# element36-io/hyperfridge-r0

Measured on AMD Instinct MI355X. Metric: segments/sec (po2=20) proving camt53 guest, 1/2/4/8 MI355X, higher is better.
Workload: dtype u32

## Files before the change

### hyperfridge-r0_amd/csrc/circuit.hpp

```cpp
#pragma once
#include <mutex>

#include "../../include/r0hip_circuit.h"
#include "internal.hpp"

namespace r0h {

struct Tap { uint32_t group, offset, back; };
struct Reg { uint32_t group, offset, first_tap, size, combo; };
struct Step { uint32_t op, a, b, c; };
struct CodeCol { uint32_t kind, param; };
struct DataCol { uint32_t kind, a, b, c, e; };
struct AccCol { uint32_t first, a, b; };
struct Term { uint32_t pow, v; std::vector<uint32_t> conds; };
struct LfTerm { uint32_t coef, global, col; };
struct Lf { std::vector<LfTerm> terms; };
struct LogupPart { uint32_t ch_kind, ch_idx; Lf lf; };
struct LogupFraction { uint32_t table; Lf num; std::vector<LogupPart> parts; };
struct LogupAcc { uint32_t final_global; std::vector<LogupFraction> fr; };
struct LogupTable { uint32_t data_col, kind; };
struct Logup {
  std::vector<LogupTable> tables;
  std::vector<LogupAcc> accs;
  uint32_t n_chain = 0;
// ... 42 lines not shown
  std::vector<uint32_t> global_cols;
  std::vector<r0h::Step> steps;
  uint32_t ret = 0;
  std::vector<uint32_t> fp_step, mix_step;
  std::vector<r0h::CodeCol> code_cols;
  std::vector<r0h::DataCol> data_cols;
  std::vector<r0h::AccCol> acc_cols;
  r0h::Logup logup;
  uint32_t period = 0;
  std::vector<uint32_t> periodic;
  bool has_sponge = false;
  uint32_t sponge_code = 0, sponge_data = 0, sponge_global = 0;
  uint32_t n_late = 0;
  bool has_column_program = false;
  std::vector<uint32_t> blob;
  uint8_t info[16] = {'R', '0', 'H', 'I', 'P', '_', 'S', 'Y', 'N', 'T', 'H', ':', 'v', '1', '_', '_'};
  r0h::Plan plan;
  hipModule_t module = nullptr;
  std::vector<hipFunction_t> kernels;
  mutable std::mutex check_mu;
  mutable hipModule_t check_module = nullptr;
  mutable std::vector<hipFunction_t> check_kernels;
};

namespace r0h {
const char* parse_blob(r0h_circuit* c, const uint32_t* blob, size_t n_words);
void make_plan(r0h_circuit* c);
std::string emit_source(const r0h_circuit* c);
std::string emit_check_source(const r0h_circuit* c);
const char* sponge_plant(r0h_ctx* ctx, const r0h_circuit* c, uint32_t po2, const uint32_t* words, size_t n_words, r0h_buf* data);
const char* require_witness(const char* caller, r0h_ctx* ctx, const r0h_circuit* c, uint32_t po2, const r0h_buf* accum, const r0h_buf* code, const r0h_buf* data,
                            const uint32_t* global, const uint32_t* mix);
const char* logup_accum(r0h_ctx* ctx, const r0h_circuit* c, uint32_t po2, const r0h_buf* code, const r0h_buf* data, const uint32_t* global, const uint32_t* mix, r0h_buf* accum);
}
```

### hyperfridge-r0_amd/csrc/fp.hpp

```cpp
#pragma once
#include <stdint.h>
#if defined(__HIPCC__)
#include <hip/hip_runtime.h>
#define R0H_HD __host__ __device__ __forceinline__
#else
#define R0H_HD inline
#endif

namespace r0h {

constexpr uint32_t P = 2013265921u;
constexpr uint32_t NPINV = 0x77ffffffu;
constexpr uint32_t R2 = 1172168163u;
constexpr uint32_t ONE = 268435454u;
constexpr uint32_t ROU_GEN = 137u;
constexpr uint32_t BETA_CANON = 11u;

R0H_HD uint32_t reduce1(uint32_t x) {
#if defined(__HIP_DEVICE_COMPILE__)
  uint32_t r;
  asm("v_subrev_co_u32 %0, vcc, 0x78000001, %1\n\tv_cndmask_b32 %0, %0, %1, vcc" : "=&v"(r) : "v"(x) : "vcc");
  return r;
#else
  uint32_t y = x - P;
  return y < x ? y : x;
#endif
}
R0H_HD uint32_t add(uint32_t a, uint32_t b) { return reduce1(a + b); }
R0H_HD uint32_t sub(uint32_t a, uint32_t b) {
#if defined(__HIP_DEVICE_COMPILE__)
  uint32_t d, e;
  asm("v_sub_co_u32 %0, vcc, %2, %3\n\tv_add_u32 %1, 0x78000001, %0\n\tv_cndmask_b32 %0, %0, %1, vcc"
      : "=&v"(d), "=&v"(e) : "v"(a), "v"(b) : "vcc");
  return d;
#else
  uint32_t d = a - b, e = d + P;
  return d < e ? d : e;
#endif
}
// ... 66 lines not shown
  uint32_t c4 = reduce64((u64)a.e[1] * b.e[3] + (u64)a.e[2] * b.e[2] + (u64)a.e[3] * b.e[1]);
  uint32_t c5 = reduce64((u64)a.e[2] * b.e[3] + (u64)a.e[3] * b.e[2]);
  uint32_t c6 = reduce64((u64)a.e[3] * b.e[3]);
  Fp4 r;
  r.e[0] = reduce64((u64)a.e[0] * b.e[0] + (u64)BETA_M * c4);
  r.e[1] = reduce64((u64)a.e[0] * b.e[1] + (u64)a.e[1] * b.e[0] + (u64)BETA_M * c5);
  r.e[2] = reduce64((u64)a.e[0] * b.e[2] + (u64)a.e[1] * b.e[1] + (u64)a.e[2] * b.e[0] + (u64)BETA_M * c6);
  r.e[3] = reduce64((u64)a.e[0] * b.e[3] + (u64)a.e[1] * b.e[2] + (u64)a.e[2] * b.e[1] + (u64)a.e[3] * b.e[0]);
  return r;
}
R0H_HD Fp4 fp4_pow(Fp4 a, uint64_t n) {
  Fp4 r = fp4_one();
  while (n) {
    if (n & 1) r = r * a;
    a = a * a;
    n >>= 1;
  }
  return r;
}
R0H_HD Fp4 fp4_inv(const Fp4& a) {
  uint32_t A0 = a.e[0], A1 = a.e[2], B0 = a.e[1], B1 = a.e[3];
  uint32_t A2_0 = add(mul(A0, A0), mul(BETA_M, mul(A1, A1))), A2_1 = mul(add(A0, A0), A1);
  uint32_t B2_0 = add(mul(B0, B0), mul(BETA_M, mul(B1, B1))), B2_1 = mul(add(B0, B0), B1);
  uint32_t D0 = sub(A2_0, mul(BETA_M, B2_1)), D1 = sub(A2_1, B2_0);
  uint32_t n = inv(sub(mul(D0, D0), mul(BETA_M, mul(D1, D1))));
  uint32_t I0 = mul(D0, n), I1 = neg(mul(D1, n));
  Fp4 r;
  r.e[0] = add(mul(A0, I0), mul(BETA_M, mul(A1, I1)));
  r.e[2] = add(mul(A0, I1), mul(A1, I0));
  r.e[1] = neg(add(mul(B0, I0), mul(BETA_M, mul(B1, I1))));
  r.e[3] = neg(add(mul(B0, I1), mul(B1, I0)));
  return r;
}

R0H_HD uint32_t bitrev(uint32_t x, uint32_t bits) {
#if defined(__HIP_DEVICE_COMPILE__)
  return bits ? __brev(x) >> (32 - bits) : 0u;
#else
  uint32_t r = 0;
  for (uint32_t i = 0; i < bits; i++) r |= ((x >> i) & 1u) << (bits - 1 - i);
  return r;
#endif
}
inline uint32_t rou_fwd(uint32_t po2) { return fpow(enc(ROU_GEN), 1ull << (27 - po2)); }
inline uint32_t rou_rev(uint32_t po2) { return inv(rou_fwd(po2)); }

}
```

### hyperfridge-r0_amd/csrc/internal.hpp

```cpp
#pragma once
#include <hip/hip_runtime.h>
#include <stdint.h>
#include <stdio.h>
#include <stdlib.h>
#include <string.h>

#include <map>
#include <memory>
#include <string>
#include <vector>

#include "../../include/r0hip.h"
#include "fp.hpp"

namespace r0h {

const char* make_error(const char* fmt, ...);

#define R0H_TRY_HIP(expr)                                                                              \
  do {                                                                                                 \
    hipError_t e__ = (expr);                                                                           \
    if (e__ != hipSuccess) return r0h::make_error("%s:%d: %s: %s", __FILE__, __LINE__, #expr, hipGetErrorString(e__)); \
  } while (0)
#define R0H_TRY(expr)                \
// ... 19 lines not shown
constexpr uint32_t TW_TOP = 22;
constexpr uint32_t TWB_BITS = 13;
constexpr uint32_t TWB_SIZE = 1u << TWB_BITS;
constexpr uint32_t MAX_DOMAIN_PO2 = 26;
constexpr size_t POOL_LIMIT = (size_t)192 << 30;

struct P2Consts {
  uint32_t rc_full[2 * P2_HALF_FULL][P2_CELLS];
  uint32_t rc_partial[P2_PARTIAL];
  uint32_t diag[P2_CELLS];
  uint32_t diag_canon[P2_CELLS];
  uint32_t diag_shoup[P2_CELLS];
  uint32_t part_sigma[P2_PART_SIGMA_WORDS];
  uint32_t part_final[(P2_CELLS - 1) * (P2_PARTIAL + 1)];
};

struct KTimer {
  std::vector<hipEvent_t> ev;
  size_t used = 0;
  double alg_bytes = 0;
};

struct Profile {
  std::vector<const char*> names;
  std::vector<float> ms;
  std::vector<hipEvent_t> events;
};

}

struct r0h_ctx {
  int device = 0;
  int refs = 1;

  hipStream_t stream = nullptr;
  uint32_t* tw_lo[2] = {nullptr, nullptr};
  uint32_t* tw_hi[2] = {nullptr, nullptr};
  uint32_t* tw12[2] = {nullptr, nullptr};
  uint32_t* twb_lo[2] = {nullptr, nullptr};
  uint32_t* twb_hi[2] = {nullptr, nullptr};
  uint32_t* pow3_lo = nullptr;
  uint32_t* pow3_hi = nullptr;
  uint32_t* pow3_top = nullptr;
  r0h::P2Consts* p2 = nullptr;
  r0h::P2Consts p2_host;
  int hashfn = 0;
  void* scratch = nullptr;
  size_t scratch_bytes = 0;
  void* pinned = nullptr;
  size_t pinned_bytes = 0, pinned_off = 0;
  std::multimap<size_t, void*> pool;
  size_t pool_bytes = 0;
  r0h::Profile prof;
  r0h_session_stats session = {0, 0, 0, 0, 0, 0, 0};
  const r0h_circuit* image_circuit = nullptr;
  uint64_t session_resident_limit = 0;
  void* session_rows = nullptr;
  std::vector<r0h_ctx*> helpers;
  bool check_witness = false;
  bool ktime_on = false;
  std::map<std::string, r0h::KTimer> ktimers;
};

struct r0h_buf {
  r0h_ctx* ctx = nullptr;
  void* ptr = nullptr;
// ... 94 lines not shown
```

### hyperfridge-r0_amd/csrc/logup.hip

```cpp
#include <algorithm>
#include <map>

#include "../../include/r0hip_circuit.h"
#include "circuit.hpp"

namespace r0h {

namespace {
struct Tape {
  std::vector<uint32_t> words;
  std::vector<const uint32_t*> cols;
  std::vector<Fp4> ch;
  std::vector<uint32_t> acc_begin;
};

const char* build_tape(const r0h_circuit* c, uint32_t po2, const r0h_buf* code, const r0h_buf* data, const uint32_t* global, const uint32_t* mix, Tape* t, bool lookups_only = false) {
  std::map<uint32_t, uint32_t> col_index;
  std::map<uint64_t, uint32_t> ch_index;
  t->ch.push_back(fp4_one());
  auto form = [&](const Lf& lf) -> const char* {
    t->words.push_back((uint32_t)lf.terms.size());
    for (const LfTerm& term : lf.terms) {
      uint32_t coef = enc(term.coef);
      if (term.global) {
        R0H_REQUIRE(global, "log-derivative accumulation: a form reads a public input and none were given");
        coef = mul(coef, global[term.global - 1]);
      }
      uint32_t col = 0;
      if (term.col) {
        const uint32_t ref = term.col - 1;
        auto it = col_index.find(ref);
        if (it == col_index.end()) {
          const r0h_buf* src = (ref >> 28) == R0H_GROUP_CODE ? code : data;
          R0H_REQUIRE(src, "log-derivative accumulation: a form reads the %s group and none was given", (ref >> 28) == R0H_GROUP_CODE ? "CODE" : "DATA");
          it = col_index.emplace(ref, (uint32_t)t->cols.size()).first;
          t->cols.push_back(u32(src) + ((size_t)(ref & 0xfffffu) << po2));
        }
        col = it->second + 1;
      }
      t->words.push_back(coef);
      t->words.push_back(col);
    }
    return nullptr;
  };
  for (const LogupAcc& a : c->logup.accs) {
    t->acc_begin.push_back((uint32_t)t->words.size());
    for (const LogupFraction& f : a.fr) {
      if (lookups_only && !f.table) continue;
      t->words.push_back(f.table);
      R0H_TRY(form(f.num));
      t->words.push_back((uint32_t)f.parts.size());
      for (const LogupPart& q : f.parts) {
        uint32_t idx = 0;
        if (q.ch_kind) {
          const uint64_t key = (uint64_t)q.ch_kind << 32 | q.ch_idx;
          auto it = ch_index.find(key);
          if (it == ch_index.end()) {
            const uint32_t* src = q.ch_kind == 1 ? mix + 4 * (size_t)q.ch_idx : global + q.ch_idx;
            R0H_REQUIRE(q.ch_kind == 1 ? mix != nullptr : global != nullptr, "log-derivative accumulation: a challenge is read from %s and none were given", q.ch_kind == 1 ? "the mix" : "the public inputs");
            it = ch_index.emplace(key, (uint32_t)t->ch.size()).first;
            t->ch.push_back(Fp4{{src[0], src[1], src[2], src[3]}});
          }
          idx = it->second;
        }
        t->words.push_back(idx);
        R0H_TRY(form(q.lf));
      }
    }
  }
  t->acc_begin.push_back((uint32_t)t->words.size());
  return nullptr;
}

struct DeviceTape {
  DevBuf buf;
  const uint32_t* words = nullptr;
  const uint32_t* const* cols = nullptr;
  const Fp4* ch = nullptr;
};
const char* upload_tape(r0h_ctx* ctx, const Tape& t, DeviceTape* d) {
  const size_t w_bytes = (t.words.size() * 4 + 15) & ~(size_t)15, c_bytes = (t.cols.size() * sizeof(void*) + 15) & ~(size_t)15, h_bytes = t.ch.size() * 16;
  R0H_TRY(d->buf.alloc(ctx, w_bytes + c_bytes + h_bytes));
  char* base = (char*)d->buf->ptr;
  R0H_TRY(stage_h2d(ctx, base, t.words.data(), t.words.size() * 4));
  R0H_TRY(stage_h2d(ctx, base + w_bytes, t.cols.data(), t.cols.size() * sizeof(void*)));
  R0H_TRY(stage_h2d(ctx, base + w_bytes + c_bytes, t.ch.data(), h_bytes));
  d->words = (const uint32_t*)base;
  d->cols = (const uint32_t* const*)(base + w_bytes);
  d->ch = (const Fp4*)(base + w_bytes + c_bytes);
  return nullptr;
}

__device__ __forceinline__ uint32_t eval_form(const uint32_t* __restrict__ tape, uint32_t& at, const uint32_t* const* __restrict__ cols, uint32_t r) {
  const uint32_t n = tape[at++];
  uint32_t acc = 0;
  for (uint32_t k = 0; k < n; k++) {
    const uint32_t coef = tape[at], col = tape[at + 1];
    at += 2;
    acc = add(acc, col ? mul(coef, cols[col - 1][r]) : coef);
  }
  return acc;
}

constexpr uint32_t HOT = 4096;

__global__ __launch_bounds__(256) void logup_count_kernel(uint32_t* __restrict__ hist , uint32_t* __restrict__ err, const uint32_t* __restrict__ tape,
                                                          uint32_t tape_end, const uint32_t* const* __restrict__ cols, uint32_t n, uint32_t n_tables) {
  __shared__ uint32_t hot[2][HOT];
  for (uint32_t i = threadIdx.x; i < 2 * HOT; i += 256) (&hot[0][0])[i] = 0;
  __syncthreads();
  const uint32_t r = blockIdx.x * 256u + threadIdx.x;
  uint32_t gated[2] = {0, 0};
  if (r < n) {
    uint32_t at = 0;
    while (at < tape_end) {
      const uint32_t table = tape[at++];
      const uint32_t num = eval_form(tape, at, cols, r);
      const uint32_t n_parts = tape[at++];
      uint32_t value = 0;
      for (uint32_t q = 0; q < n_parts; q++) {
        at++;
        const uint32_t v = eval_form(tape, at, cols, r);
        if (q == 1) value = v;
      }
      if (!table || table > n_tables) continue;
      if (num != ONE) {
        if (num) atomicOr(err, 1u);
        else gated[table - 1]++;
        continue;
      }
      uint32_t v = dec(neg(value));
      if (table == R0H_TABLE_AND) {
        v -= R0H_TAG_AND;
        if (v >> 24 || ((v & 255u) & ((v >> 8) & 255u)) != v >> 16) { atomicOr(err, 2u); continue; }
        v &= 0xffffu;
      } else if (v >> 16) {
        atomicOr(err, 2u);
        continue;
      }
      if (!v) continue;
      if (v < HOT) atomicAdd(&hot[table - 1][v], 1u);
      else atomicAdd(&hist[(size_t)(table - 1) * 65536 + v], 1u);
    }
  }
  if (gated[0]) atomicAdd(&hot[0][0], gated[0]);
  if (gated[1]) atomicAdd(&hot[1][0], gated[1]);
  __syncthreads();
  for (uint32_t i = threadIdx.x; i < 2 * HOT; i += 256) {
    const uint32_t cnt = (&hot[0][0])[i];
    if (cnt) atomicAdd(&hist[(size_t)(i / HOT) * 65536 + (i % HOT)], cnt);
  }
}
__global__ void logup_mult_kernel(uint32_t* __restrict__ column, const uint32_t* __restrict__ hist, uint32_t total, uint32_t n) {
  __shared__ uint32_t part[256];
  const uint32_t r = blockIdx.x * 256u + threadIdx.x;
  if (blockIdx.x == 0) {
    uint32_t s = 0;
    for (uint32_t i = threadIdx.x; i < 65536u; i += 256) s += hist[i];
    part[threadIdx.x] = s;
    __syncthreads();
    for (uint32_t k = 128; k; k >>= 1) {
      if (threadIdx.x < k) part[threadIdx.x] += part[threadIdx.x + k];
      __syncthreads();
    }
  }
  if (r >= n) return;
  uint32_t v = r < 65536u ? hist[r] : 0u;
  if (r == 0) v = total - part[0];
  column[r] = enc(v);
}

__global__ __launch_bounds__(256) void logup_term_kernel(uint32_t* __restrict__ accum, uint32_t* __restrict__ row_total, uint32_t* __restrict__ own_terms,
                                                         const uint32_t* __restrict__ tape, const uint32_t* const* __restrict__ cols, const Fp4* __restrict__ ch,
                                                         uint32_t a0, uint32_t a1, uint32_t n_chain, uint32_t po2) {
  const uint32_t r = blockIdx.x * 256u + threadIdx.x, n = 1u << po2;
  if (r >= n) return;
  uint32_t at = 0;
  Fp4 run = fp4_zero();
  for (uint32_t j = a0; j < a1; j++) {
    Fp4 d[4];
    uint32_t num[4];
    for (uint32_t f = 0; f < 4; f++) {
      at++;
      num[f] = eval_form(tape, at, cols, r);
      const uint32_t n_parts = tape[at++];
      Fp4 den = fp4_zero();
      for (uint32_t q = 0; q < n_parts; q++) {
        const uint32_t ci = tape[at++];
        const uint32_t v = eval_form(tape, at, cols, r);
        if (ci == 0) den.e[0] = add(den.e[0], v);
        else den = den + scale(ch[ci], v);
      }
      d[f] = den;
    }
    const Fp4 d01 = d[0] * d[1], d23 = d[2] * d[3];
    const Fp4 top = (scale(d[1], num[0]) + scale(d[0], num[1])) * d23 + (scale(d[3], num[2]) + scale(d[2], num[3])) * d01;
    const Fp4 term = top * fp4_inv(d01 * d23);
    if (j < n_chain) {
      run = run + term;
      for (uint32_t i = 0; i < 4; i++) accum[((size_t)(4 * j + i) << po2) + r] = run.e[i];
    } else {
      *(uint4*)(own_terms + 4 * ((size_t)(j - n_chain) * n + r)) = make_uint4(term.e[0], term.e[1], term.e[2], term.e[3]);
    }
  }
  if (a0 < n_chain) *(uint4*)(row_total + 4 * (size_t)r) = make_uint4(run.e[0], run.e[1], run.e[2], run.e[3]);
}
__global__ void logup_chain_kernel(uint32_t* __restrict__ accum, const uint32_t* __restrict__ scanned, uint32_t n_cols, uint32_t po2) {
  const uint32_t r = blockIdx.x * 256u + threadIdx.x, col = blockIdx.y;
  if (r == 0 || r >= (1u << po2) || col >= n_cols) return;
  uint32_t* cell = accum + ((size_t)col << po2) + r;
  *cell = add(*cell, scanned[4 * (size_t)(r - 1) + (col & 3u)]);
}
}

static const char* own_accumulators(r0h_ctx* ctx, const r0h_circuit* c, uint32_t po2, const Tape& t, const DeviceTape& d, r0h_buf* accum, uint32_t* totals_out) {
  const uint32_t n = 1u << po2, n_chain = c->logup.n_chain, n_acc = (uint32_t)c->logup.accs.size(), n_own = n_acc - n_chain;
  if (!n_own) return nullptr;
  DevBuf terms;
  R0H_TRY(terms.alloc(ctx, (size_t)n_own * n * 16));
  hipLaunchKernelGGL(logup_term_kernel, dim3((n + 255) / 256), dim3(256), 0, ctx->stream, accum ? u32(accum) : nullptr, (uint32_t*)nullptr, u32(terms.get()),
                     d.words + t.acc_begin[n_chain], d.cols, d.ch, n_chain, n_acc, n_chain, po2);
  R0H_TRY(launch_ok("logup_term_kernel"));
  for (uint32_t k = 0; k < n_own; k++) {
    r0h_buf view = buf_view(terms.get(), (size_t)k * n * 16, (size_t)n * 16);
    R0H_TRY(r0h_prefix_sums(ctx, &view, n));
    if (accum) R0H_TRY(unpack_ext_columns(ctx, u32(accum) + ((size_t)(4 * (n_chain + k)) << po2), (const uint32_t*)view.ptr, po2));
    if (totals_out) R0H_TRY(r0h_buf_d2h(ctx, &view, (size_t)(n - 1) * 16, totals_out + 4 * k, 16));
  }
  return nullptr;
}

const char* logup_accum(r0h_ctx* ctx, const r0h_circuit* c, uint32_t po2, const r0h_buf* code, const r0h_buf* data, const uint32_t* global, const uint32_t* mix, r0h_buf* accum) {
  R0H_GUARD_BEGIN
  R0H_REQUIRE(ctx && c && data && accum, "r0h_accum: NULL argument");
  R0H_REQUIRE(po2 >= 4 && po2 <= R0H_MAX_PO2, "r0h_accum: po2 %u outside [4, %u]", po2, R0H_MAX_PO2);
  const uint32_t n = 1u << po2, n_chain = c->logup.n_chain;
  R0H_REQUIRE(((size_t)c->group_size[R0H_GROUP_DATA] << po2) * 4 <= data->bytes && ((size_t)c->group_size[R0H_GROUP_ACCUM] << po2) * 4 <= accum->bytes &&
                  (!code || ((size_t)c->group_size[R0H_GROUP_CODE] << po2) * 4 <= code->bytes),
              "r0h_accum: buffers too small for 2^%u rows", po2);
  for (uint32_t i = 0; i < c->n_mix; i++) R0H_REQUIRE(mix && mix[i] < P, "r0h_accum: mix[%u] missing or not canonical", i);
  for (uint32_t i = 0; i < c->n_global; i++) R0H_REQUIRE(!global || global[i] < P, "r0h_accum: global[%u] not canonical", i);
  Tape t;
  R0H_TRY(build_tape(c, po2, code, data, global, mix, &t));
  DeviceTape d;
  R0H_TRY(upload_tape(ctx, t, &d));
  KScope ks(ctx, "logup_accum", ((double)t.cols.size() + 2.0 * c->group_size[R0H_GROUP_ACCUM]) * n * 4);
  DevBuf totals;
  R0H_TRY(totals.alloc(ctx, (size_t)n * 16));
  hipLaunchKernelGGL(logup_term_kernel, dim3((n + 255) / 256), dim3(256), 0, ctx->stream, u32(accum), u32(totals.get()), (uint32_t*)nullptr, d.words, d.cols, d.ch, 0u, n_chain, n_chain, po2);
  R0H_TRY(launch_ok("logup_term_kernel"));
  R0H_TRY(r0h_prefix_sums(ctx, totals.get(), n));
  hipLaunchKernelGGL(logup_chain_kernel, dim3((n + 255) / 256, 4 * n_chain), dim3(256), 0, ctx->stream, u32(accum), u32(totals.get()), 4 * n_chain, po2);
  R0H_TRY(launch_ok("logup_chain_kernel"));
  R0H_TRY(own_accumulators(ctx, c, po2, t, d, accum, nullptr));
  R0H_TRY_HIP(hipStreamSynchronize(ctx->stream));
  return nullptr;
  R0H_GUARD_END
}

}

using namespace r0h;

extern "C" {

const char* r0h_logup_multiplicities(r0h_ctx* ctx, const r0h_circuit* c, uint32_t po2, r0h_buf* data, const uint32_t* global) {
  R0H_GUARD_BEGIN
  R0H_REQUIRE(ctx && c && data, "r0h_logup_multiplicities: NULL argument");
  if (c->logup.tables.empty()) return nullptr;
  R0H_REQUIRE(po2 >= 16 && po2 <= R0H_MAX_PO2, "r0h_logup_multiplicities: the tables have 2^16 rows: po2 %u outside [16, %u]", po2, R0H_MAX_PO2);
  R0H_REQUIRE(((size_t)c->group_size[R0H_GROUP_DATA] << po2) * 4 <= data->bytes, "r0h_logup_multiplicities: the DATA buffer is too small for 2^%u rows", po2);
  R0H_REQUIRE(c->logup.tables.size() <= 2, "r0h_logup_multiplicities: at most two tables");
  const uint32_t n = 1u << po2, n_tables = (uint32_t)c->logup.tables.size();
  Tape t;
  std::vector<uint32_t> dummy_mix(c->n_mix, 0), dummy_global(c->n_global, 0);
  R0H_TRY(build_tape(c, po2, nullptr, data, global ? global : dummy_global.data(), dummy_mix.data(), &t, true));
  DeviceTape d;
  R0H_TRY(upload_tape(ctx, t, &d));
  std::vector<uint64_t> slots(n_tables, 0);
  for (uint32_t j = 0; j < c->logup.n_chain; j++)
    for (const LogupFraction& f : c->logup.accs[j].fr)
      if (f.table && f.table <= n_tables) slots[f.table - 1] += n;
  for (uint32_t k = 0; k < n_tables; k++)
    R0H_REQUIRE(slots[k] <= P - 1, "r0h_logup_multiplicities: table %u has %llu lookup slots at 2^%u rows: more than p - 1", k, (unsigned long long)slots[k], po2);
  DevBuf hist;
  const size_t hist_words = (size_t)n_tables * 65536;
  R0H_TRY(hist.alloc(ctx, hist_words * 4 + 16));
  R0H_TRY_HIP(hipMemsetAsync(hist->ptr, 0, hist_words * 4 + 16, ctx->stream));
  KScope ks(ctx, "logup_multiplicities", (double)t.cols.size() * n * 4);
  hipLaunchKernelGGL(logup_count_kernel, dim3((n + 255) / 256), dim3(256), 0, ctx->stream, u32(hist.get()), u32(hist.get()) + hist_words, d.words, (uint32_t)t.words.size(), d.cols, n, n_tables);
  R0H_TRY(launch_ok("logup_count_kernel"));
  for (uint32_t k = 0; k < n_tables; k++) {
    const LogupTable& tb = c->logup.tables[k];
    hipLaunchKernelGGL(logup_mult_kernel, dim3((n + 255) / 256), dim3(256), 0, ctx->stream, u32(data) + ((size_t)tb.data_col << po2), u32(hist.get()) + (size_t)k * 65536,
                       (uint32_t)slots[k], n);
    R0H_TRY(launch_ok("logup_mult_kernel"));
  }
  R0H_TRY_HIP(hipStreamSynchronize(ctx->stream));
  uint32_t err = 0;
  R0H_TRY(r0h_buf_d2h(ctx, hist.get(), hist_words * 4, &err, 4));
  R0H_REQUIRE(!(err & 1u), "r0h_logup_multiplicities: a lookup's numerator is neither 0 nor 1");
  R0H_REQUIRE(!(err & 2u), "r0h_logup_multiplicities: a row whose numerator is 1 looks up a value that is not in its table");
  return nullptr;
  R0H_GUARD_END
}

const char* r0h_logup_totals(r0h_ctx* ctx, const r0h_circuit* c, uint32_t po2, const r0h_buf* code, const r0h_buf* data, uint32_t* global_io) {
  R0H_GUARD_BEGIN
  R0H_REQUIRE(ctx && c && data && global_io, "r0h_logup_totals: NULL argument");
  R0H_REQUIRE(po2 >= 4 && po2 <= R0H_MAX_PO2, "r0h_logup_totals: po2 %u outside [4, %u]", po2, R0H_MAX_PO2);
  const uint32_t n_chain = c->logup.n_chain, n_acc = (uint32_t)c->logup.accs.size();
  if (n_acc == n_chain) return nullptr;
  for (uint32_t j = n_chain; j < n_acc; j++)
    for (const LogupFraction& f : c->logup.accs[j].fr)
      for (const LogupPart& q : f.parts) R0H_REQUIRE(q.ch_kind != 1, "r0h_logup_totals: accumulator %u takes a challenge from the mix", j);
  Tape t;
  std::vector<uint32_t> dummy_mix(c->n_mix, 0);
  R0H_TRY(build_tape(c, po2, code ? code : data, data, global_io, dummy_mix.data(), &t));
  DeviceTape d;
  R0H_TRY(upload_tape(ctx, t, &d));
  std::vector<uint32_t> totals(4 * (size_t)(n_acc - n_chain));
  R0H_TRY(own_accumulators(ctx, c, po2, t, d, nullptr, totals.data()));
  for (uint32_t j = n_chain; j < n_acc; j++) memcpy(global_io + c->logup.accs[j].final_global, totals.data() + 4 * (size_t)(j - n_chain), 16);
  return nullptr;
  R0H_GUARD_END
}

}
```

### hyperfridge-r0_amd/csrc/logup_host.cpp

```cpp
#include <string.h>

#include <vector>

#include "../../include/r0hip_circuit.h"
#include "circuit.hpp"

using namespace r0h;

extern "C" {

const char* r0h_logup_multiplicities_host(const uint32_t* blob, size_t blob_words, uint32_t po2, uint32_t* data, const uint32_t* global) {
  R0H_GUARD_BEGIN
  R0H_REQUIRE(blob && data, "r0h_logup_multiplicities_host: NULL argument");
  r0h_circuit c;
  R0H_TRY(parse_blob(&c, blob, blob_words));
  if (c.logup.tables.empty()) return nullptr;
  R0H_REQUIRE(po2 >= 16 && po2 <= R0H_MAX_PO2, "r0h_logup_multiplicities_host: the tables have 2^16 rows: po2 %u outside [16, %u]", po2, (unsigned)R0H_MAX_PO2);
  const size_t n = (size_t)1 << po2;
  std::vector<std::vector<uint32_t>> hist(c.logup.tables.size(), std::vector<uint32_t>(65536, 0));
  std::vector<uint64_t> slots(c.logup.tables.size(), 0);
  for (uint32_t j = 0; j < c.logup.n_chain; j++)
    for (const LogupFraction& f : c.logup.accs[j].fr)
      if (f.table) slots[f.table - 1] += n;
  for (size_t k = 0; k < slots.size(); k++)
    R0H_REQUIRE(slots[k] <= P - 1, "r0h_logup_multiplicities_host: table %zu has %llu lookup slots at 2^%u rows: more than p - 1", k, (unsigned long long)slots[k], po2);
  auto form = [&](const Lf& lf, size_t r) {
    uint32_t acc = 0;
    for (const LfTerm& t : lf.terms) {
      uint32_t v = enc(t.coef);
      if (t.global) v = mul(v, global ? global[t.global - 1] : 0u);
      if (t.col) v = mul(v, data[(size_t)((t.col - 1) & 0xfffffu) * n + r]);
      acc = add(acc, v);
    }
    return acc;
  };
  for (uint32_t j = 0; j < c.logup.n_chain; j++)
    for (const LogupFraction& f : c.logup.accs[j].fr) {
      if (!f.table) continue;
      for (size_t r = 0; r < n; r++) {
        const uint32_t num = form(f.num, r);
// ... 24 lines not shown
```

### hyperfridge-r0_amd/csrc/session.cpp

```cpp
#include <stdlib.h>
#include <string.h>

#include <algorithm>
#include <atomic>
#include <chrono>
#include <condition_variable>
#include <deque>
#include <map>
#include <memory>
#include <mutex>
#include <thread>
#include <utility>
#include <vector>

#include "circuit.hpp"
#include "receipt_types.hpp"

using namespace r0h;

namespace {
using Clock = std::chrono::steady_clock;
double seconds(Clock::time_point a, Clock::time_point b) { return std::chrono::duration<double>(b - a).count(); }

struct CodeCommits {
// ... 467 lines not shown
  R0H_TRY(r0h_vm_journal(run.vm, &journal, &journal_len));
  ses->journal.assign(journal, journal + journal_len);
  system_state_digest(run.first_pre, ses->image_id);
  ses->stats.cycles = ses->cycles;
  ses->stats.executor_s = run.executor_s;
  *session_out = ses.release();
  return nullptr;
  R0H_GUARD_END
}

size_t r0h_session_n_segments(const r0h_session* s) { return s ? s->n_segments : 0; }

const char* r0h_session_records(const r0h_session* s, uint32_t* indices_out, uint32_t* records_out, size_t capacity, size_t* n_out) {
  R0H_REQUIRE(s && n_out, "r0h_session_records: NULL argument");
  *n_out = s->trace_mode ? s->pending.size() : 0;
  if (!s->trace_mode) return nullptr;
  R0H_REQUIRE(capacity >= s->pending.size() && indices_out && records_out, "r0h_session_records: room for %zu records wanted", s->pending.size());
  const uint32_t n_early = R0H_TRACE_GLOBALS - R0H_TRACE_LATE_GLOBALS;
  for (size_t k = 0; k < s->pending.size(); k++) {
    indices_out[k] = (uint32_t)s->pending[k].index;
    memcpy(records_out + k * RECORD_WORDS, s->pending[k].global.data(), n_early * 4);
    memcpy(records_out + k * RECORD_WORDS + n_early, s->pending[k].root, 32);
  }
  return nullptr;
}

namespace {
const char* finish_segment(r0h_session* s, Pending& p, const uint32_t challenge[16], std::vector<uint32_t>& mix, std::vector<uint32_t>& seal, size_t* words) {
  const r0h_circuit* c = s->c;
  DevBuf data = std::move(p.data);
  memcpy(p.global.data() + R0H_TRACE_GAMMA, challenge, 64);
  const r0h_buf* code_cols = nullptr;
  R0H_TRY(r0h_code_commit_columns(p.cc, &code_cols));
  R0H_TRY(r0h_logup_totals(p.lctx, c, p.po2, code_cols, data.get(), p.global.data()));
  R0H_TRY(r0h_proof_late(p.proof.get(), p.global.data() + (R0H_TRACE_GLOBALS - R0H_TRACE_LATE_GLOBALS), mix.data()));
  DevBuf accum;
  R0H_TRY(accum.alloc(p.lctx, ((size_t)c->group_size[R0H_GROUP_ACCUM] << p.po2) * 4));
  R0H_TRY(r0h_accum_public(p.lctx, c, p.po2, code_cols, data.get(), p.global.data(), mix.data(), accum.get()));
  return r0h_proof_finish(p.proof.release(), accum.get(), seal.data(), seal.size(), words);
}
}

const char* r0h_session_finish(r0h_session* s, const uint32_t* all_records, size_t n_records, r0h_receipt** receipt_out, uint8_t image_id_out[32], uint64_t* cycles_out) {
  R0H_GUARD_BEGIN
  R0H_REQUIRE(s && receipt_out, "r0h_session_finish: NULL argument");
  std::vector<uint32_t> image_seal;
  if (s->trace_mode) {
    R0H_REQUIRE(all_records && n_records == s->n_segments, "r0h_session_finish: the session has %zu segments, %zu records were given", s->n_segments, n_records);
    const uint32_t n_early = R0H_TRACE_GLOBALS - R0H_TRACE_LATE_GLOBALS;
    for (const Pending& p : s->pending)
      R0H_REQUIRE(!memcmp(all_records + p.index * RECORD_WORDS, p.global.data(), n_early * 4) && !memcmp(all_records + p.index * RECORD_WORDS + n_early, p.root, 32),
                  "r0h_session_finish: record %zu is not the one this rank committed", p.index);
    uint32_t challenge[16];
    session_challenge(all_records, n_records, challenge);
    std::atomic<bool> failed(false);
    auto lane = [&](r0h_ctx* lctx) -> const char* {
      std::vector<uint32_t> seal((size_t)1 << 20), mix(s->c->n_mix);
      size_t words = 0;
      if (lctx == s->ctx && !s->elf.empty() && s->ctx->image_circuit) {
        R0H_TRY(r0h_prove_image(s->ctx, s->ctx->image_circuit, s->elf.data(), s->elf.size(), challenge, seal.data(), seal.size(), &words));
        image_seal.assign(seal.begin(), seal.begin() + words);
      }
      for (Pending& p : s->pending) {
        if (p.lctx != lctx || p.done) continue;
        if (failed) return nullptr;
        const Clock::time_point t0 = Clock::now();
        R0H_TRY(finish_segment(s, p, challenge, mix, seal, &words));
        std::lock_guard<std::mutex> lk(s->result_mu);
        p.seal.assign(seal.begin(), seal.begin() + words);
        p.done = true;
        s->stats.prove_ms += 1e3 * seconds(t0, Clock::now());
// ... 54 lines not shown
```

Before: 40.68.

## Batch logup inversions, reuse kept own-accumulator terms, rewrite multiplicity histogram

The term kernel now evaluates up to four accumulators and shares a single Fp4 inversion across them with Montgomery batch inversion. The own-accumulator terms computed during the totals pass are kept and unpacked into the accumulator buffer at finish, so the second evaluation is skipped. The multiplicity counter now reads a compact per-table lookup list instead of the full tape and uses a persistent grid with 32K-bin shared histograms split into two halves. In exchange it holds an extra device buffer between the two phases and makes two passes per table in the count kernel.

```diff
diff --git a/hyperfridge-r0_amd/csrc/circuit.hpp b/hyperfridge-r0_amd/csrc/circuit.hpp
--- a/hyperfridge-r0_amd/csrc/circuit.hpp
+++ b/hyperfridge-r0_amd/csrc/circuit.hpp
@@ -98,4 +98,17 @@
 const char* require_witness(const char* caller, r0h_ctx* ctx, const r0h_circuit* c, uint32_t po2, const r0h_buf* accum, const r0h_buf* code, const r0h_buf* data,
                             const uint32_t* global, const uint32_t* mix);
 const char* logup_accum(r0h_ctx* ctx, const r0h_circuit* c, uint32_t po2, const r0h_buf* code, const r0h_buf* data, const uint32_t* global, const uint32_t* mix, r0h_buf* accum);
+struct LogupKept {
+  DevBuf terms;
+  uint32_t po2 = 0, n_own = 0;
+};
+const char* logup_totals_keep(r0h_ctx* ctx, const r0h_circuit* c, uint32_t po2, const r0h_buf* code, const r0h_buf* data, uint32_t* global_io, LogupKept* keep);
+const char* logup_accum_kept(r0h_ctx* ctx, const r0h_circuit* c, uint32_t po2, const r0h_buf* code, const r0h_buf* data, const uint32_t* global, const uint32_t* mix, r0h_buf* accum,
+                             const LogupKept* kept);
+struct LookupList {
+  std::vector<uint32_t> words;
+  uint32_t begin[3] = {0, 0, 0}, entries[2] = {0, 0};
+  uint32_t n_cols = 0;
+};
+const char* logup_lookup_list(const r0h_circuit* c, const uint32_t* global, LookupList* out);
 }
diff --git a/hyperfridge-r0_amd/csrc/fp.hpp b/hyperfridge-r0_amd/csrc/fp.hpp
--- a/hyperfridge-r0_amd/csrc/fp.hpp
+++ b/hyperfridge-r0_amd/csrc/fp.hpp
@@ -5,6 +5,11 @@
 #define R0H_HD __host__ __device__ __forceinline__
 #else
 #define R0H_HD inline
+#endif
+#if defined(__clang__)
+#define R0H_UNROLL _Pragma("unroll")
+#else
+#define R0H_UNROLL
 #endif
 
 namespace r0h {
@@ -137,6 +142,26 @@
   r.e[3] = neg(add(mul(B0, I1), mul(B1, I0)));
   return r;
 }
+template <int NB>
+R0H_HD void fp4_batch_div(Fp4 (&top)[NB], const Fp4 (&den)[NB]) {
+  Fp4 d[NB], before[NB];
+  bool zero[NB];
+  Fp4 run = fp4_one();
+R0H_UNROLL
+  for (int k = 0; k < NB; k++) {
+    zero[k] = (den[k].e[0] | den[k].e[1] | den[k].e[2] | den[k].e[3]) == 0;
+    d[k] = zero[k] ? fp4_one() : den[k];
+    before[k] = run;
+    run = k ? run * d[k] : d[k];
+  }
+  Fp4 inv_run = fp4_inv(run);
+R0H_UNROLL
+  for (int k = NB - 1; k >= 0; k--) {
+    const Fp4 inv_k = k ? inv_run * before[k] : inv_run;
+    if (k) inv_run = inv_run * d[k];
+    top[k] = zero[k] ? fp4_zero() : top[k] * inv_k;
+  }
+}
 
 R0H_HD uint32_t bitrev(uint32_t x, uint32_t bits) {
 #if defined(__HIP_DEVICE_COMPILE__)
diff --git a/hyperfridge-r0_amd/csrc/internal.hpp b/hyperfridge-r0_amd/csrc/internal.hpp
--- a/hyperfridge-r0_amd/csrc/internal.hpp
+++ b/hyperfridge-r0_amd/csrc/internal.hpp
@@ -75,6 +75,7 @@
 struct r0h_ctx {
   int device = 0;
   int refs = 1;
+  int n_cu = 0;
 
   hipStream_t stream = nullptr;
   uint32_t* tw_lo[2] = {nullptr, nullptr};
diff --git a/hyperfridge-r0_amd/csrc/logup.hip b/hyperfridge-r0_amd/csrc/logup.hip
--- a/hyperfridge-r0_amd/csrc/logup.hip
+++ b/hyperfridge-r0_amd/csrc/logup.hip
@@ -14,7 +14,7 @@
   std::vector<uint32_t> acc_begin;
 };
 
-const char* build_tape(const r0h_circuit* c, uint32_t po2, const r0h_buf* code, const r0h_buf* data, const uint32_t* global, const uint32_t* mix, Tape* t, bool lookups_only = false) {
+const char* build_tape(const r0h_circuit* c, uint32_t po2, const r0h_buf* code, const r0h_buf* data, const uint32_t* global, const uint32_t* mix, Tape* t) {
   std::map<uint32_t, uint32_t> col_index;
   std::map<uint64_t, uint32_t> ch_index;
   t->ch.push_back(fp4_one());
@@ -46,7 +46,6 @@
   for (const LogupAcc& a : c->logup.accs) {
     t->acc_begin.push_back((uint32_t)t->words.size());
     for (const LogupFraction& f : a.fr) {
-      if (lookups_only && !f.table) continue;
       t->words.push_back(f.table);
       R0H_TRY(form(f.num));
       t->words.push_back((uint32_t)f.parts.size());
@@ -102,74 +101,116 @@
   return acc;
 }
 
-constexpr uint32_t HOT = 4096;
-
-__global__ __launch_bounds__(256) void logup_count_kernel(uint32_t* __restrict__ hist , uint32_t* __restrict__ err, const uint32_t* __restrict__ tape,
-                                                          uint32_t tape_end, const uint32_t* const* __restrict__ cols, uint32_t n, uint32_t n_tables) {
-  __shared__ uint32_t hot[2][HOT];
-  for (uint32_t i = threadIdx.x; i < 2 * HOT; i += 256) (&hot[0][0])[i] = 0;
+__device__ __forceinline__ uint32_t eval_list_form(const uint32_t* __restrict__ list, uint32_t& at, const uint32_t* __restrict__ data, uint32_t po2, uint32_t r) {
+  const uint32_t n = list[at++];
+  uint32_t acc = 0;
+  for (uint32_t k = 0; k < n; k++) {
+    const uint32_t coef = list[at], col = list[at + 1];
+    at += 2;
+    acc = add(acc, col ? mul(coef, data[((size_t)(col - 1) << po2) + r]) : coef);
+  }
+  return acc;
+}
+
+constexpr uint32_t BINS = 32768;
+constexpr uint32_t COUNT_THREADS = 1024;
+
+__global__ __launch_bounds__(COUNT_THREADS) void logup_count_kernel(uint32_t* __restrict__ hist , uint32_t* __restrict__ counters, uint32_t* __restrict__ err,
+                                                                    const uint32_t* __restrict__ list, uint32_t n_entries, const uint32_t* __restrict__ data, uint32_t po2,
+                                                                    uint32_t half, uint32_t is_and) {
+  __shared__ uint32_t bins[BINS];
+  __shared__ uint32_t sums[2];
+  for (uint32_t i = threadIdx.x; i < BINS; i += COUNT_THREADS) bins[i] = 0;
+  if (threadIdx.x < 2) sums[threadIdx.x] = 0;
   __syncthreads();
-  const uint32_t r = blockIdx.x * 256u + threadIdx.x;
-  uint32_t gated[2] = {0, 0};
-  if (r < n) {
+  const uint32_t n = 1u << po2, lo = half * BINS;
+  uint32_t gated = 0, bad = 0;
+  for (uint32_t r = blockIdx.x * COUNT_THREADS + threadIdx.x; r < n; r += gridDim.x * COUNT_THREADS) {
     uint32_t at = 0;
-    while (at < tape_end) {
-      const uint32_t table = tape[at++];
-      const uint32_t num = eval_form(tape, at, cols, r);
-      const uint32_t n_parts = tape[at++];
-      uint32_t value = 0;
-      for (uint32_t q = 0; q < n_parts; q++) {
-        at++;
-        const uint32_t v = eval_form(tape, at, cols, r);
-        if (q == 1) value = v;
-      }
-      if (!table || table > n_tables) continue;
+    for (uint32_t e = 0; e < n_entries; e++) {
+      const uint32_t num = eval_list_form(list, at, data, po2, r);
+      const uint32_t value = eval_list_form(list, at, data, po2, r);
       if (num != ONE) {
-        if (num) atomicOr(err, 1u);
-        else gated[table - 1]++;
+        if (num) bad |= 1u;
+        else gated++;
         continue;
       }
       uint32_t v = dec(neg(value));
-      if (table == R0H_TABLE_AND) {
+      if (is_and) {
         v -= R0H_TAG_AND;
-        if (v >> 24 || ((v & 255u) & ((v >> 8) & 255u)) != v >> 16) { atomicOr(err, 2u); continue; }
+        if (v >> 24 || ((v & 255u) & ((v >> 8) & 255u)) != v >> 16) { bad |= 2u; continue; }
         v &= 0xffffu;
       } else if (v >> 16) {
-        atomicOr(err, 2u);
+        bad |= 2u;
         continue;
       }
-      if (!v) continue;
-      if (v < HOT) atomicAdd(&hot[table - 1][v], 1u);
-      else atomicAdd(&hist[(size_t)(table - 1) * 65536 + v], 1u);
-    }
-  }
-  if (gated[0]) atomicAdd(&hot[0][0], gated[0]);
-  if (gated[1]) atomicAdd(&hot[1][0], gated[1]);
+      if (v && v - lo < BINS) atomicAdd(&bins[v - lo], 1u);
+    }
+  }
+  if (bad) atomicOr(err, bad);
   __syncthreads();
-  for (uint32_t i = threadIdx.x; i < 2 * HOT; i += 256) {
-    const uint32_t cnt = (&hot[0][0])[i];
-    if (cnt) atomicAdd(&hist[(size_t)(i / HOT) * 65536 + (i % HOT)], cnt);
-  }
-}
-__global__ void logup_mult_kernel(uint32_t* __restrict__ column, const uint32_t* __restrict__ hist, uint32_t total, uint32_t n) {
-  __shared__ uint32_t part[256];
+  uint32_t binned = 0;
+  for (uint32_t i = threadIdx.x; i < BINS; i += COUNT_THREADS) {
+    const uint32_t cnt = bins[i];
+    if (cnt) atomicAdd(&hist[lo + i], cnt);
+    binned += cnt;
+  }
+  if (binned) atomicAdd(&sums[0], binned);
+  if (gated && half == 0) atomicAdd(&sums[1], gated);
+  __syncthreads();
+  if (threadIdx.x < 2 && sums[threadIdx.x]) atomicAdd(&counters[threadIdx.x], sums[threadIdx.x]);
+}
+__global__ void logup_mult_kernel(uint32_t* __restrict__ column, const uint32_t* __restrict__ hist, const uint32_t* __restrict__ counters, uint32_t total, uint32_t n) {
   const uint32_t r = blockIdx.x * 256u + threadIdx.x;
-  if (blockIdx.x == 0) {
-    uint32_t s = 0;
-    for (uint32_t i = threadIdx.x; i < 65536u; i += 256) s += hist[i];
-    part[threadIdx.x] = s;
-    __syncthreads();
-    for (uint32_t k = 128; k; k >>= 1) {
-      if (threadIdx.x < k) part[threadIdx.x] += part[threadIdx.x + k];
-      __syncthreads();
-    }
-  }
   if (r >= n) return;
   uint32_t v = r < 65536u ? hist[r] : 0u;
-  if (r == 0) v = total - part[0];
+  if (r == 0) v = total - counters[0] - counters[1];
   column[r] = enc(v);
 }
 
+__device__ __forceinline__ void eval_accumulator(const uint32_t* __restrict__ tape, uint32_t& at, const uint32_t* const* __restrict__ cols, const Fp4* __restrict__ ch, uint32_t r,
+                                                 Fp4& top, Fp4& den_out) {
+  Fp4 d[4];
+  uint32_t num[4];
+#pragma unroll
+  for (uint32_t f = 0; f < 4; f++) {
+    at++;
+    num[f] = eval_form(tape, at, cols, r);
+    const uint32_t n_parts = tape[at++];
+    Fp4 den = fp4_zero();
+    for (uint32_t q = 0; q < n_parts; q++) {
+      const uint32_t ci = tape[at++];
+      const uint32_t v = eval_form(tape, at, cols, r);
+      if (ci == 0) den.e[0] = add(den.e[0], v);
+      else den = den + scale(ch[ci], v);
+    }
+    d[f] = den;
+  }
+  const Fp4 d01 = d[0] * d[1], d23 = d[2] * d[3];
+  top = (scale(d[1], num[0]) + scale(d[0], num[1])) * d23 + (scale(d[3], num[2]) + scale(d[2], num[3])) * d01;
+  den_out = d01 * d23;
+}
+template <int NB>
+__device__ __forceinline__ void term_batch(uint32_t* __restrict__ accum, uint32_t* __restrict__ own_terms, const uint32_t* __restrict__ tape, uint32_t& at,
+                                           const uint32_t* const* __restrict__ cols, const Fp4* __restrict__ ch, uint32_t j, uint32_t n_chain, uint32_t po2, uint32_t r, Fp4& run) {
+  Fp4 top[NB], den[NB];
+  eval_accumulator(tape, at, cols, ch, r, top[0], den[0]);
+  if constexpr (NB > 1) eval_accumulator(tape, at, cols, ch, r, top[1], den[1]);
+  if constexpr (NB > 2) eval_accumulator(tape, at, cols, ch, r, top[2], den[2]);
+  if constexpr (NB > 3) eval_accumulator(tape, at, cols, ch, r, top[3], den[3]);
+  static_assert(NB >= 1 && NB <= 4, "batches of one to four accumulators");
+  fp4_batch_div<NB>(top, den);
+#pragma unroll
+  for (int k = 0; k < NB; k++) {
+    const Fp4 term = top[k];
+    if (j + k < n_chain) {
+      run = run + term;
+      for (uint32_t i = 0; i < 4; i++) accum[((size_t)(4 * (j + k) + i) << po2) + r] = run.e[i];
+    } else {
+      *(uint4*)(own_terms + 4 * (((size_t)(j + k - n_chain) << po2) + r)) = make_uint4(term.e[0], term.e[1], term.e[2], term.e[3]);
+    }
+  }
+}
 __global__ __launch_bounds__(256) void logup_term_kernel(uint32_t* __restrict__ accum, uint32_t* __restrict__ row_total, uint32_t* __restrict__ own_terms,
                                                          const uint32_t* __restrict__ tape, const uint32_t* const* __restrict__ cols, const Fp4* __restrict__ ch,
                                                          uint32_t a0, uint32_t a1, uint32_t n_chain, uint32_t po2) {
@@ -177,32 +218,11 @@
   if (r >= n) return;
   uint32_t at = 0;
   Fp4 run = fp4_zero();
-  for (uint32_t j = a0; j < a1; j++) {
-    Fp4 d[4];
-    uint32_t num[4];
-    for (uint32_t f = 0; f < 4; f++) {
-      at++;
-      num[f] = eval_form(tape, at, cols, r);
-      const uint32_t n_parts = tape[at++];
-      Fp4 den = fp4_zero();
-      for (uint32_t q = 0; q < n_parts; q++) {
-        const uint32_t ci = tape[at++];
-        const uint32_t v = eval_form(tape, at, cols, r);
-        if (ci == 0) den.e[0] = add(den.e[0], v);
-        else den = den + scale(ch[ci], v);
-      }
-      d[f] = den;
-    }
-    const Fp4 d01 = d[0] * d[1], d23 = d[2] * d[3];
-    const Fp4 top = (scale(d[1], num[0]) + scale(d[0], num[1])) * d23 + (scale(d[3], num[2]) + scale(d[2], num[3])) * d01;
-    const Fp4 term = top * fp4_inv(d01 * d23);
-    if (j < n_chain) {
-      run = run + term;
-      for (uint32_t i = 0; i < 4; i++) accum[((size_t)(4 * j + i) << po2) + r] = run.e[i];
-    } else {
-      *(uint4*)(own_terms + 4 * ((size_t)(j - n_chain) * n + r)) = make_uint4(term.e[0], term.e[1], term.e[2], term.e[3]);
-    }
-  }
+  uint32_t j = a0;
+  for (; j + 4 <= a1; j += 4) term_batch<4>(accum, own_terms, tape, at, cols, ch, j, n_chain, po2, r, run);
+  if (a1 - j == 3) term_batch<3>(accum, own_terms, tape, at, cols, ch, j, n_chain, po2, r, run);
+  else if (a1 - j == 2) term_batch<2>(accum, own_terms, tape, at, cols, ch, j, n_chain, po2, r, run);
+  else if (a1 - j == 1) term_batch<1>(accum, own_terms, tape, at, cols, ch, j, n_chain, po2, r, run);
   if (a0 < n_chain) *(uint4*)(row_total + 4 * (size_t)r) = make_uint4(run.e[0], run.e[1], run.e[2], run.e[3]);
 }
 __global__ void logup_chain_kernel(uint32_t* __restrict__ accum, const uint32_t* __restrict__ scanned, uint32_t n_cols, uint32_t po2) {
@@ -213,7 +233,9 @@
 }
 }
 
-static const char* own_accumulators(r0h_ctx* ctx, const r0h_circuit* c, uint32_t po2, const Tape& t, const DeviceTape& d, r0h_buf* accum, uint32_t* totals_out) {
+static_assert(sizeof(DevBuf) == sizeof(void*) && sizeof(LogupKept) == sizeof(void*) + 8 && alignof(LogupKept) == alignof(void*),
+              "LogupKept is no longer {buffer pointer, po2, n_own}: tests/test_gpu_logup_kept.py builds one by hand");
+static const char* own_accumulators(r0h_ctx* ctx, const r0h_circuit* c, uint32_t po2, const Tape& t, const DeviceTape& d, r0h_buf* accum, uint32_t* totals_out, LogupKept* keep = nullptr) {
   const uint32_t n = 1u << po2, n_chain = c->logup.n_chain, n_acc = (uint32_t)c->logup.accs.size(), n_own = n_acc - n_chain;
   if (!n_own) return nullptr;
   DevBuf terms;
@@ -227,10 +249,20 @@
     if (accum) R0H_TRY(unpack_ext_columns(ctx, u32(accum) + ((size_t)(4 * (n_chain + k)) << po2), (const uint32_t*)view.ptr, po2));
     if (totals_out) R0H_TRY(r0h_buf_d2h(ctx, &view, (size_t)(n - 1) * 16, totals_out + 4 * k, 16));
   }
+  if (keep) {
+    keep->terms = std::move(terms);
+    keep->po2 = po2;
+    keep->n_own = n_own;
+  }
   return nullptr;
 }
 
 const char* logup_accum(r0h_ctx* ctx, const r0h_circuit* c, uint32_t po2, const r0h_buf* code, const r0h_buf* data, const uint32_t* global, const uint32_t* mix, r0h_buf* accum) {
+  return logup_accum_kept(ctx, c, po2, code, data, global, mix, accum, nullptr);
+}
+
+const char* logup_accum_kept(r0h_ctx* ctx, const r0h_circuit* c, uint32_t po2, const r0h_buf* code, const r0h_buf* data, const uint32_t* global, const uint32_t* mix, r0h_buf* accum,
+                             const LogupKept* kept) {
   R0H_GUARD_BEGIN
   R0H_REQUIRE(ctx && c && data && accum, "r0h_accum: NULL argument");
   R0H_REQUIRE(po2 >= 4 && po2 <= R0H_MAX_PO2, "r0h_accum: po2 %u outside [4, %u]", po2, R0H_MAX_PO2);
@@ -252,7 +284,14 @@
   R0H_TRY(r0h_prefix_sums(ctx, totals.get(), n));
   hipLaunchKernelGGL(logup_chain_kernel, dim3((n + 255) / 256, 4 * n_chain), dim3(256), 0, ctx->stream, u32(accum), u32(totals.get()), 4 * n_chain, po2);
   R0H_TRY(launch_ok("logup_chain_kernel"));
-  R0H_TRY(own_accumulators(ctx, c, po2, t, d, accum, nullptr));
+  if (kept && kept->terms) {
+    const uint32_t n_own = (uint32_t)c->logup.accs.size() - n_chain;
+    R0H_REQUIRE(kept->po2 == po2 && kept->n_own == n_own && kept->terms->ctx == ctx, "r0h_accum: the kept terms are not this segment's (2^%u rows, %u accumulators)", kept->po2, kept->n_own);
+    for (uint32_t k = 0; k < n_own; k++)
+      R0H_TRY(unpack_ext_columns(ctx, u32(accum) + ((size_t)(4 * (n_chain + k)) << po2), u32(kept->terms.get()) + 4 * (size_t)k * n, po2));
+  } else {
+    R0H_TRY(own_accumulators(ctx, c, po2, t, d, accum, nullptr));
+  }
   R0H_TRY_HIP(hipStreamSynchronize(ctx->stream));
   return nullptr;
   R0H_GUARD_END
@@ -272,33 +311,38 @@
   R0H_REQUIRE(((size_t)c->group_size[R0H_GROUP_DATA] << po2) * 4 <= data->bytes, "r0h_logup_multiplicities: the DATA buffer is too small for 2^%u rows", po2);
   R0H_REQUIRE(c->logup.tables.size() <= 2, "r0h_logup_multiplicities: at most two tables");
   const uint32_t n = 1u << po2, n_tables = (uint32_t)c->logup.tables.size();
-  Tape t;
-  std::vector<uint32_t> dummy_mix(c->n_mix, 0), dummy_global(c->n_global, 0);
-  R0H_TRY(build_tape(c, po2, nullptr, data, global ? global : dummy_global.data(), dummy_mix.data(), &t, true));
-  DeviceTape d;
-  R0H_TRY(upload_tape(ctx, t, &d));
+  LookupList list;
+  R0H_TRY(logup_lookup_list(c, global, &list));
   std::vector<uint64_t> slots(n_tables, 0);
-  for (uint32_t j = 0; j < c->logup.n_chain; j++)
-    for (const LogupFraction& f : c->logup.accs[j].fr)
-      if (f.table && f.table <= n_tables) slots[f.table - 1] += n;
+  for (uint32_t k = 0; k < n_tables; k++) slots[k] = (uint64_t)list.entries[k] * n;
   for (uint32_t k = 0; k < n_tables; k++)
     R0H_REQUIRE(slots[k] <= P - 1, "r0h_logup_multiplicities: table %u has %llu lookup slots at 2^%u rows: more than p - 1", k, (unsigned long long)slots[k], po2);
+  DevBuf dlist;
+  R0H_TRY(dlist.alloc(ctx, list.words.size() * 4 + 16));
+  R0H_TRY(stage_h2d(ctx, dlist->ptr, list.words.data(), list.words.size() * 4));
   DevBuf hist;
   const size_t hist_words = (size_t)n_tables * 65536;
-  R0H_TRY(hist.alloc(ctx, hist_words * 4 + 16));
-  R0H_TRY_HIP(hipMemsetAsync(hist->ptr, 0, hist_words * 4 + 16, ctx->stream));
-  KScope ks(ctx, "logup_multiplicities", (double)t.cols.size() * n * 4);
-  hipLaunchKernelGGL(logup_count_kernel, dim3((n + 255) / 256), dim3(256), 0, ctx->stream, u32(hist.get()), u32(hist.get()) + hist_words, d.words, (uint32_t)t.words.size(), d.cols, n, n_tables);
-  R0H_TRY(launch_ok("logup_count_kernel"));
+  R0H_TRY(hist.alloc(ctx, hist_words * 4 + 32));
+  R0H_TRY_HIP(hipMemsetAsync(hist->ptr, 0, hist_words * 4 + 32, ctx->stream));
+  uint32_t* const counters = u32(hist.get()) + hist_words;
+  uint32_t* const err_word = counters + 4;
+  if (!ctx->n_cu) R0H_TRY_HIP(hipDeviceGetAttribute(&ctx->n_cu, hipDeviceAttributeMultiprocessorCount, ctx->device));
+  const uint32_t grid = std::min<uint32_t>((uint32_t)std::max(ctx->n_cu, 1), n / COUNT_THREADS);
+  KScope ks(ctx, "logup_multiplicities", 2.0 * list.n_cols * n * 4);
   for (uint32_t k = 0; k < n_tables; k++) {
+    for (uint32_t half = 0; half < 2; half++) {
+      hipLaunchKernelGGL(logup_count_kernel, dim3(grid), dim3(COUNT_THREADS), 0, ctx->stream, u32(hist.get()) + (size_t)k * 65536, counters + 2 * k, err_word, u32(dlist.get()) + list.begin[k],
+                         list.entries[k], u32(data), po2, half, (uint32_t)(k + 1 == R0H_TABLE_AND));
+      R0H_TRY(launch_ok("logup_count_kernel"));
+    }
     const LogupTable& tb = c->logup.tables[k];
-    hipLaunchKernelGGL(logup_mult_kernel, dim3((n + 255) / 256), dim3(256), 0, ctx->stream, u32(data) + ((size_t)tb.data_col << po2), u32(hist.get()) + (size_t)k * 65536,
+    hipLaunchKernelGGL(logup_mult_kernel, dim3((n + 255) / 256), dim3(256), 0, ctx->stream, u32(data) + ((size_t)tb.data_col << po2), u32(hist.get()) + (size_t)k * 65536, counters + 2 * k,
                        (uint32_t)slots[k], n);
     R0H_TRY(launch_ok("logup_mult_kernel"));
   }
   R0H_TRY_HIP(hipStreamSynchronize(ctx->stream));
   uint32_t err = 0;
-  R0H_TRY(r0h_buf_d2h(ctx, hist.get(), hist_words * 4, &err, 4));
+  R0H_TRY(r0h_buf_d2h(ctx, hist.get(), hist_words * 4 + 16, &err, 4));
   R0H_REQUIRE(!(err & 1u), "r0h_logup_multiplicities: a lookup's numerator is neither 0 nor 1");
   R0H_REQUIRE(!(err & 2u), "r0h_logup_multiplicities: a row whose numerator is 1 looks up a value that is not in its table");
   return nullptr;
@@ -306,6 +350,12 @@
 }
 
 const char* r0h_logup_totals(r0h_ctx* ctx, const r0h_circuit* c, uint32_t po2, const r0h_buf* code, const r0h_buf* data, uint32_t* global_io) {
+  return logup_totals_keep(ctx, c, po2, code, data, global_io, nullptr);
+}
+
+}
+
+const char* r0h::logup_totals_keep(r0h_ctx* ctx, const r0h_circuit* c, uint32_t po2, const r0h_buf* code, const r0h_buf* data, uint32_t* global_io, LogupKept* keep) {
   R0H_GUARD_BEGIN
   R0H_REQUIRE(ctx && c && data && global_io, "r0h_logup_totals: NULL argument");
   R0H_REQUIRE(po2 >= 4 && po2 <= R0H_MAX_PO2, "r0h_logup_totals: po2 %u outside [4, %u]", po2, R0H_MAX_PO2);
@@ -320,10 +370,8 @@
   DeviceTape d;
   R0H_TRY(upload_tape(ctx, t, &d));
   std::vector<uint32_t> totals(4 * (size_t)(n_acc - n_chain));
-  R0H_TRY(own_accumulators(ctx, c, po2, t, d, nullptr, totals.data()));
+  R0H_TRY(own_accumulators(ctx, c, po2, t, d, nullptr, totals.data(), keep));
   for (uint32_t j = n_chain; j < n_acc; j++) memcpy(global_io + c->logup.accs[j].final_global, totals.data() + 4 * (size_t)(j - n_chain), 16);
   return nullptr;
   R0H_GUARD_END
 }
-
-}
diff --git a/hyperfridge-r0_amd/csrc/logup_host.cpp b/hyperfridge-r0_amd/csrc/logup_host.cpp
--- a/hyperfridge-r0_amd/csrc/logup_host.cpp
+++ b/hyperfridge-r0_amd/csrc/logup_host.cpp
@@ -5,7 +5,39 @@
 #include "../../include/r0hip_circuit.h"
 #include "circuit.hpp"
 
+#include <set>
+
 using namespace r0h;
+
+namespace r0h {
+const char* logup_lookup_list(const r0h_circuit* c, const uint32_t* global, LookupList* out) {
+  R0H_REQUIRE(c->logup.tables.size() <= 2, "r0h_logup_multiplicities: at most two tables");
+  std::set<uint32_t> cols;
+  auto form = [&](const Lf& lf) {
+    out->words.push_back((uint32_t)lf.terms.size());
+    for (const LfTerm& t : lf.terms) {
+      uint32_t coef = enc(t.coef);
+      if (t.global) coef = mul(coef, global ? global[t.global - 1] : 0u);
+      out->words.push_back(coef);
+      out->words.push_back(t.col ? ((t.col - 1) & 0xfffffu) + 1 : 0u);
+      if (t.col) cols.insert((t.col - 1) & 0xfffffu);
+    }
+  };
+  for (uint32_t k = 0; k < c->logup.tables.size(); k++) {
+    out->begin[k] = (uint32_t)out->words.size();
+    for (uint32_t j = 0; j < c->logup.n_chain; j++)
+      for (const LogupFraction& f : c->logup.accs[j].fr) {
+        if (f.table != k + 1) continue;
+        form(f.num);
+        form(f.parts[1].lf);
+        out->entries[k]++;
+      }
+    out->begin[k + 1] = (uint32_t)out->words.size();
+  }
+  out->n_cols = (uint32_t)cols.size();
+  return nullptr;
+}
+}
 
 extern "C" {
 
diff --git a/hyperfridge-r0_amd/csrc/session.cpp b/hyperfridge-r0_amd/csrc/session.cpp
--- a/hyperfridge-r0_amd/csrc/session.cpp
+++ b/hyperfridge-r0_amd/csrc/session.cpp
@@ -523,11 +523,13 @@
   memcpy(p.global.data() + R0H_TRACE_GAMMA, challenge, 64);
   const r0h_buf* code_cols = nullptr;
   R0H_TRY(r0h_code_commit_columns(p.cc, &code_cols));
-  R0H_TRY(r0h_logup_totals(p.lctx, c, p.po2, code_cols, data.get(), p.global.data()));
+  LogupKept kept;
+  R0H_TRY(logup_totals_keep(p.lctx, c, p.po2, code_cols, data.get(), p.global.data(), &kept));
   R0H_TRY(r0h_proof_late(p.proof.get(), p.global.data() + (R0H_TRACE_GLOBALS - R0H_TRACE_LATE_GLOBALS), mix.data()));
   DevBuf accum;
   R0H_TRY(accum.alloc(p.lctx, ((size_t)c->group_size[R0H_GROUP_ACCUM] << p.po2) * 4));
-  R0H_TRY(r0h_accum_public(p.lctx, c, p.po2, code_cols, data.get(), p.global.data(), mix.data(), accum.get()));
+  R0H_TRY(logup_accum_kept(p.lctx, c, p.po2, code_cols, data.get(), p.global.data(), mix.data(), accum.get(), &kept));
+  kept.terms.reset();
   return r0h_proof_finish(p.proof.release(), accum.get(), seal.data(), seal.size(), words);
 }
 }
```

Result: faster. 41.63, median of 6 (+2.3%).
